# KyleVanMeter/MVOLPS

Hardware: AMD Instinct MI355X
Metric: simplex_pivots_per_s (higher is better)
Workload: dtype f64

## Files before the change

### include/mvx.h

```cpp
#ifndef MVX_H
#define MVX_H

#ifdef __cplusplus
extern "C" {
#endif

#define MVX_MIN 1
#define MVX_MAX 2
#define MVX_CV 1
#define MVX_IV 2
#define MVX_BV 3
#define MVX_FR 1
#define MVX_LO 2
#define MVX_UP 3
#define MVX_DB 4
#define MVX_FX 5
#define MVX_BS 1
#define MVX_NL 2
#define MVX_NU 3
#define MVX_NF 4
#define MVX_NS 5
#define MVX_UNDEF 1
#define MVX_FEAS 2
#define MVX_INFEAS 3
// ... 75 lines not shown
int mvx_gmi_cuts_many(const mvx_prob *const *Ps, int repaired, const int *cols, int count, double *vals, double *rhs, int *ok);
int mvx_classify_many(const mvx_prob *const *Ps, int count, int quirks, int *status, int *nviol, int *viol, double *xviol, int cap);
int mvx_branch_penalties_many(const mvx_prob *const *Ps, int count, const int *cols, const int *col_off, double tol, double *pen_down,
                              double *pen_up, int *arg_down, int *arg_up);
int mvx_round_many(const mvx_prob *root, const mvx_prob *const *Ps, int count, int mode, double *obj, int *found, double *x);
int mvx_rc_tighten_many(const mvx_prob *const *Ps, int count, const double *cutoff, double tol, int *cnt, int *cols, double *lb,
                        double *ub);
int mvx_tighten_cols_many(mvx_prob *const *Ps, int count, const int *off, const int *cols, const double *lb, const double *ub);

int mvx_get_tableau_ld(const mvx_prob *P);
int mvx_get_tableau(const mvx_prob *P, double *out);
int mvx_get_basis(const mvx_prob *P, int *head, int *nb, int *flag);

int mvx_device_count(void);
int mvx_set_device(int dev);
void mvx_profile_enable(int on);
void mvx_profile_reset(void);
double mvx_profile_update_ms(void);
long long mvx_profile_update_launches(void);
double mvx_last_solve_ms(const mvx_prob *P);
long long mvx_pack_size(const mvx_prob *P);
int mvx_pack(const mvx_prob *P, void *dev_buf);
long long mvx_pack_size_from(const mvx_prob *P, const mvx_prob *base);
int mvx_pack_from(const mvx_prob *P, const mvx_prob *base, void *dev_buf);
int mvx_unpack(mvx_prob *dst, const mvx_prob *base, const void *dev_buf);
void mvx_set_tuning(int tr, int hot, int nt);
void mvx_set_refresh(int check_every, double tol);
int mvx_get_refresh_cnt(const mvx_prob *P);
double mvx_row_residual(const mvx_prob *P);
void mvx_set_persist(int mode);
void mvx_set_chain(int len);
void mvx_set_cluster(int on);
void mvx_cluster_stats(long long *launches, long long *aborts);
void mvx_set_dual_chain(int len);
void mvx_persist_stats(long long *launches, long long *aborts);
void mvx_persist_cycles(unsigned long long *out5);
void mvx_set_batch_slots(int slots);
void mvx_sync(void);
int mvx_last_error(void);
int mvx_bind_thread(void);

#ifdef __cplusplus
}
#endif
#endif
```

### mvolps_amd/__init__.py

```python
import ctypes as C
import os

from . import capi

_HERE = os.path.dirname(os.path.abspath(__file__))
LIB_PATH = os.path.join(_HERE, "lib", "libmvolps_amd.so")

_EXTRA = {
    "device_count": (C.c_int, []),
    "set_device": (C.c_int, [C.c_int]),
    "profile_enable": (None, [C.c_int]),
    "profile_reset": (None, []),
    "profile_update_ms": (C.c_double, []),
    "profile_update_launches": (C.c_longlong, []),
    "last_solve_ms": (C.c_double, [C.c_void_p]),
    "sync": (None, []),
    "set_tuning": (None, [C.c_int, C.c_int, C.c_int]),
    "set_batch_slots": (None, [C.c_int]),
    "set_persist": (None, [C.c_int]),
    "set_chain": (None, [C.c_int]),
    "set_cluster": (None, [C.c_int]),
    "cluster_stats": (None, [C.POINTER(C.c_longlong), C.POINTER(C.c_longlong)]),
    "set_dual_chain": (None, [C.c_int]),
    "set_refresh": (None, [C.c_int, C.c_double]),
    "get_refresh_cnt": (C.c_int, [C.c_void_p]),
    "row_residual": (C.c_double, [C.c_void_p]),
    "persist_stats": (None, [C.POINTER(C.c_longlong), C.POINTER(C.c_longlong)]),
    "last_error": (C.c_int, []),
    "bind_thread": (C.c_int, []),
    "persist_cycles": (None, [C.POINTER(C.c_ulonglong)]),
    "simplex_batch": (C.c_int, [C.POINTER(C.c_void_p), C.c_int, C.c_void_p, C.POINTER(C.c_int)]),
    "pack_size": (C.c_longlong, [C.c_void_p]),
    "pack": (C.c_int, [C.c_void_p, C.c_void_p]),
    "pack_size_from": (C.c_longlong, [C.c_void_p, C.c_void_p]),
    "pack_from": (C.c_int, [C.c_void_p, C.c_void_p, C.c_void_p]),
    "unpack": (C.c_int, [C.c_void_p, C.c_void_p, C.c_void_p]),
}

_api = None


def load_library():
    if os.environ.get("MVX_NO_TORCH") != "1":
        try:
            import torch
        except Exception:
            pass
    if not os.path.exists(LIB_PATH):
        raise RuntimeError(
            "libmvolps_amd.so is missing (%s): build it with `python -m mvolps_amd.build`; "
            "there is no fallback path" % LIB_PATH
        )
    return C.CDLL(LIB_PATH)


# ... 19 lines not shown
```

### mvolps_amd/csrc/capi.cpp

```cpp
#include <cfloat>
#include <cmath>
#include <cstdio>
#include <cstdlib>
#include <chrono>
#include <cstring>

#include "engine.hpp"
#include "../../include/mvx_dist.h"

using mvx::RowPtr;

static const double INF = HUGE_VAL;
static int g_term_out = 1;

static void fault(const char *msg) {
  std::fprintf(stderr, "mvx: %s\n", msg);
  std::abort();
}

static void norm_bounds(int type, double lb, double ub, double *olb, double *oub) {
  switch (type) {
    case MVX_FR: *olb = -INF; *oub = INF; break;
    case MVX_LO: *olb = lb; *oub = INF; break;
    case MVX_UP: *olb = -INF; *oub = ub; break;
// ... 471 lines not shown
int mvx_rc_tighten_many(const mvx_prob *const *Ps, int count, const double *cutoff, double tol, int *cnt, int *cols, double *lb,
                        double *ub) {
  return mvx::engine_rc_tighten_many(Ps, count, cutoff, tol, cnt, cols, lb, ub);
}
int mvx_tighten_cols_many(mvx_prob *const *Ps, int count, const int *off, const int *cols, const double *lb, const double *ub) {
  return mvx::engine_tighten_many(Ps, count, off, cols, lb, ub);
}

int mvx_device_count(void) { return mvx::device_count(); }
int mvx_set_device(int dev) { return mvx::set_device(dev); }
long long mvx_pack_size(const mvx_prob *P) { return mvx::engine_pack_size(P, P->m); }
int mvx_pack(const mvx_prob *P, void *dev_buf) { return mvx::engine_pack(P, P->m, dev_buf); }
long long mvx_pack_size_from(const mvx_prob *P, const mvx_prob *base) { return mvx::engine_pack_size(P, base ? base->m : P->m); }
int mvx_pack_from(const mvx_prob *P, const mvx_prob *base, void *dev_buf) { return mvx::engine_pack(P, base ? base->m : P->m, dev_buf); }
int mvx_unpack(mvx_prob *dst, const mvx_prob *base, const void *dev_buf) {
  if (dst == base) return -1;
  mvx::release_device(dst);
  dst->m = base->m; dst->n = base->n; dst->dir = base->dir;
  dst->A = base->A; dst->c = base->c; dst->kind = base->kind; dst->cname = base->cname;
  dst->rtype = base->rtype; dst->rlb = base->rlb; dst->rub = base->rub;
  dst->ctype = base->ctype; dst->clb = base->clb; dst->cub = base->cub;
  dst->valid = false; dst->sol_fresh = false; dst->fresh_rows = -1;
  return mvx::engine_unpack(dst, dev_buf);
}
void mvx_set_tuning(int tr, int hot, int nt) { mvx::tuning(tr, hot, nt); }
void mvx_set_stall_limit(int limit) { mvx::set_stall_limit(limit); }
int mvx_fcs_debug_stamps(unsigned long long *out) { return mvx::fcs_debug_stamps(out); }
void mvx_set_refresh(int check_every, double tol) { mvx::set_refresh(check_every, tol); }
int mvx_get_refresh_cnt(const mvx_prob *P) { return P->refresh_cnt; }
double mvx_row_residual(const mvx_prob *P) { return mvx::row_residual(P); }
void mvx_set_persist(int mode) { mvx::set_persist(mode); }
void mvx_set_chain(int len) { mvx::set_chain(len); }
void mvx_set_cluster(int on) { mvx::set_cluster(on); }
void mvx_cluster_stats(long long *launches, long long *aborts) { mvx::cluster_stats(launches, aborts); }
void mvx_set_dual_chain(int len) { mvx::set_dual_chain(len); }
void mvx_persist_stats(long long *launches, long long *aborts) { mvx::persist_stats(launches, aborts); }
void mvx_persist_cycles(unsigned long long *out5) { mvx::persist_cycles(out5); }
void mvx_set_batch_slots(int slots) { mvx::set_batch_slots(slots); }
void mvx_profile_enable(int on) { mvx::profile_enable(on); }
void mvx_profile_reset(void) { mvx::profile_reset(); }
double mvx_profile_update_ms(void) { return mvx::profile_update_ms(); }
long long mvx_profile_update_launches(void) { return mvx::profile_update_launches(); }
double mvx_last_solve_ms(const mvx_prob *P) { return P->last_ms; }
void mvx_sync(void) { mvx::sync_stream(); }
int mvx_last_error(void) { return mvx::take_last_error(); }
int mvx_bind_thread(void) { return mvx::bind_thread(); }

void *mvx_image_alloc(size_t bytes) { return mvx::engine_image_alloc(bytes); }
void mvx_image_free(void *buf) { mvx::engine_image_free(buf); }
static long long img_pack_size(const void *P, const void *base) { return mvx_pack_size_from((const mvx_prob *)P, (const mvx_prob *)base); }
static int img_pack(const void *P, const void *base, void *buf) { return mvx_pack_from((const mvx_prob *)P, (const mvx_prob *)base, buf); }
static int img_unpack(void *dst, const void *base, const void *buf) { return mvx_unpack((mvx_prob *)dst, (const mvx_prob *)base, buf); }
const mvx_image_api *mvx_hip_image_api(void) {
  static const mvx_image_api t = {img_pack_size, img_pack, img_unpack, mvx_image_alloc, mvx_image_free};
  return &t;
}

}
```

### mvolps_amd/csrc/engine.cpp

```cpp
#include <hip/hip_runtime.h>

#include <cmath>
#include <cstdio>
#include <cstdlib>
#include <cstring>
#include <atomic>
#include <map>
#include <mutex>
#include <tuple>
#include <unordered_map>
#include <vector>

#include "engine.hpp"

struct DevMatrix {
  int m0 = 0, n = 0, lda = 0;
  double *plain = nullptr, *packed = nullptr;
  int *len = nullptr;
  std::vector<const void *> rows;
  ~DevMatrix() {
    if (packed && packed != plain) (void)hipFree(packed);
    if (plain) (void)hipFree(plain);
    if (len) (void)hipFree(len);
  }
};

struct RoundModel {
  int m0 = 0, n = 0, ldm = 0, dir = 0;
  void *dev = nullptr;
  size_t o_rlo = 0, o_rhi = 0, o_clo = 0, o_chi = 0, o_c = 0, o_flags = 0;
  std::vector<mvx::RowPtr> rows;
  std::vector<double> c, clb, cub, rlb, rub;
  std::vector<int> kind;
  ~RoundModel() {
    if (dev) (void)hipFree(dev);
  }
};

namespace mvx {

#define HIPCHECK(expr)                                                                         \
  do {                                                                                         \
    hipError_t e_ = (expr);                                                                    \
    if (e_ != hipSuccess) {                                                                    \
      std::fprintf(stderr, "mvx: HIP error %s at %s:%d (%s)\n", hipGetErrorString(e_), __FILE__, __LINE__, #expr); \
      std::abort();                                                                            \
    }                                                                                          \
  } while (0)

void set_tuning(int tr, int hot, int nt);
int fused_npb(int n);
int fused_nrb_max(int m);
int chain_ncb(int n);
int chain_nrb(int m);
void launch_pboot(const ChainArgs &, hipStream_t);
void launch_pstep(const ChainArgs &, int g, hipStream_t);
void launch_pc(const ChainArgs &, int g, hipStream_t);
void launch_fbc3(const ChainArgs &, int steps, hipStream_t);
void launch_fpatch(const ChainArgs &, int steps, hipStream_t);
int launch_chain(const ChainArgs &, hipStream_t);
int chain_cluster_nw(int m, int n);
int chain_cluster_kmax(int m, int n);
void launch_dboot(Ctl *, int n, hipStream_t);
void launch_da(Ctl *, int n, hipStream_t);
void launch_db(Ctl *, int m, int n, hipStream_t);
void launch_select(Ctl *, hipStream_t, int slots = 1);
int launch_dsel(Ctl *, int m, int n, hipStream_t, int slots = 1);
void launch_select_queue(Ctl *, const BatchQueue &q, hipStream_t, int slots);
void launch_update(Ctl *, int m, int n, hipStream_t, int slots = 1, int chained = 0, int busy_slots = 0);
void launch_p1_head(Ctl *, hipStream_t);
void launch_p1_select(Ctl *, hipStream_t);
void launch_p1_fix(Ctl *, int n, hipStream_t);
void launch_scatter_ctl(Ctl *dst, const Ctl *src, const int *idx, int count, hipStream_t);
void launch_copy_many(const CopyBatch &b, hipStream_t);
void launch_gmi(const GmiArgs &a, hipStream_t);
void launch_classify(const ClsArgs &a, hipStream_t);
void launch_penalty(const PenArgs &a, hipStream_t);
void launch_round(const RndArgs &a, hipStream_t);
void launch_rcfix(const RcArgs &a, hipStream_t);
void launch_tighten(const TightHandle *hs, const TightEntry *es, int count, hipStream_t);
void launch_refresh_select(Ctl *, const int *tflag, int var, hipStream_t);
size_t persist_lds_bytes(int m, int cpw);
int persist_max_cpw();
int persist_slot_words(int m_cap);
int launch_persist(Ctl *, unsigned long long *head, unsigned long long *slot, int *abort_flag, unsigned long long *dbg, int m, int cpw, int nw,
                   int slot_stride, int max_steps, int head_stride, hipStream_t);
void launch_rowcomb(Ctl *, int m, int n, int respect_done, hipStream_t);
void launch_shift_nonbasic(double *T, int ld, int m, int jj, double delta, hipStream_t);
void launch_set_basic_bounds(double *blb, double *bub, int i, double lb, double ub, hipStream_t);
void launch_set_nonbasic(double *nlb, double *nub, int *nflag, int j, double lb, double ub, int flag, hipStream_t);
void launch_add_rows(double *T, int ld, int n, int *bvar, double *blb, double *bub, int *nvar, int first, int nrs, int m_new,
// ... 543 lines not shown
    default: return MVX_NS;
  }
}

static void rebuild_pos(mvx_prob *P) {
  P->pos.assign((size_t)P->m + P->n + 1, 0);
  for (int i = 1; i <= P->m; i++) P->pos[P->bvar[i]] = i;
  for (int j = 1; j <= P->n; j++) P->pos[P->nvar[j]] = -j;
}

static inline void var_bounds(const mvx_prob *P, int k, double *lb, double *ub) {
  if (k <= P->m) {
    *lb = P->rlb[k];
    *ub = P->rub[k];
  } else {
    *lb = P->clb[k - P->m];
    *ub = P->cub[k - P->m];
  }
}

static std::atomic<int> g_cluster{-1};
static std::atomic<bool> g_cluster_broken{false};
static std::atomic<long long> g_cluster_launches{0}, g_cluster_aborts{0};
static bool cluster_wanted() {
  int v = g_cluster.load();
  if (v < 0) {
    const char *e = std::getenv("MVX_CLUSTER");
    v = e ? (std::atoi(e) != 0) : 1;
    g_cluster.store(v);
  }
  return v != 0 && !g_cluster_broken.load();
}

static int g_chain = -1;
static int chain_length(const mvx_prob *P) {
  if (g_chain < 0) {
    const char *e = std::getenv("MVX_CHAIN");
    g_chain = e ? std::max(1, std::min(KCH, std::atoi(e))) : 0;
  }
  if (g_chain > 0) return g_chain;
  const size_t bytes = (size_t)(P->m + 1) * (size_t)P->ld * 8;
  if (cluster_wanted() && chain_cluster_kmax(P->m, P->n) > 0) return bytes < ((size_t)24 << 20) ? 16 : 32;
  if (bytes < ((size_t)24 << 20)) return 8;
  return 16;
}

static int g_dchain = -1;
static int dual_chain_length(bool wide, bool on_chip = false) {
  if (g_dchain < 0) {
    const char *e = std::getenv("MVX_DCHAIN");
    g_dchain = e ? std::max(1, std::min(DCH_MAX, std::atoi(e))) : 0;
  }
  if (g_dchain > 0) return g_dchain;
  if (on_chip) return 8;
  return wide ? 8 : 4;
}

static void fill_ctl(SolveCtx &sc, mvx_prob *P, Ctl *h) {
  std::memset(h, 0, sizeof(Ctl));
  h->T = P->d_T;
  h->bvar = P->d_bvar; h->blb = P->d_blb; h->bub = P->d_bub;
  h->nvar = P->d_nvar; h->nflag = P->d_nflag; h->nlb = P->d_nlb; h->nub = P->d_nub;
  h->colq = sc.d_colq; h->srow = sc.d_srow; h->cost1 = sc.d_cost1; h->wts = sc.d_wts;
  h->gflag = sc.d_gflag; h->part = sc.d_part; h->rc_base = nullptr; h->rc_out = sc.d_cost1;
  h->m = P->m; h->n = P->n; h->ld = P->ld; h->m_cap = P->m_cap;
  h->sgn = (P->dir == MVX_MAX) ? 1.0 : -1.0;
// ... 364 lines not shown
    if (J.profiled) HIPCHECK(hipEventRecord(c.ev_pool[J.ev_used++], sc.stream));
  };
  int depth;
  if (J.try_fused) depth = std::max(0, std::min(batch, remaining));
  else depth = std::max(1, std::min(batch, remaining));
  auto body = [&](int m_grid) {
    if (J.try_fused) {
      PersistPlan pl;
      if (depth > 0 && !J.profiled && J.resident && !(J.cluster && !g_cluster_broken.load()) && persist_plan(c, P, &pl) && ensure_persist(c, sc, P, pl)) {
        launch_select(sc.d_ctl, sc.stream);
        launch_update(sc.d_ctl, m_grid, n, sc.stream, 1, 1);
        HIPCHECK(hipMemcpyAsync(sc.p_backup, P->slab, P->slab_bytes, hipMemcpyDeviceToDevice, sc.stream));
        HIPCHECK(hipMemcpyAsync(sc.d_pctl, sc.d_ctl, sizeof(Ctl), hipMemcpyDeviceToDevice, sc.stream));
        HIPCHECK(hipMemcpyAsync(sc.d_ppw, sc.d_pw[0], (size_t)P->ld * 8, hipMemcpyDeviceToDevice, sc.stream));
        HIPCHECK(hipMemcpyAsync(sc.d_ppw + P->ld, sc.d_pw[1], (size_t)P->ld * 8, hipMemcpyDeviceToDevice, sc.stream));
        const int head_stride = 4;
        HIPCHECK(hipMemsetAsync(sc.d_pcand, 0, (size_t)2 * pl.nw * head_stride * 8, sc.stream));
        const int steps = 1 << 24;
        if (launch_persist(sc.d_ctl, sc.d_pcand, sc.d_pmsg, sc.d_pabort, (unsigned long long *)(sc.d_pabort + 16), P->m, pl.cpw, pl.nw, sc.p_msg_words, steps, head_stride, sc.stream) == 0) {
          J.persist_queued = true;
          g_persist_launches++;
          launch_select(sc.d_ctl, sc.stream);
          launch_update(sc.d_ctl, m_grid, n, sc.stream, 1, 1);
        } else {
          g_persist_broken = true;
        }
      } else {
        const size_t e_generic = J.ev_used;
        if (J.profiled) J.ev_used += 2;
        if (depth > 0) {
          const bool cl = J.cluster && !g_cluster_broken.load();
          if (!cl) launch_pboot(J.cargs, sc.stream);
          bool first = true;
          const int kc = cl ? std::max(1, std::min(J.chain0, chain_cluster_kmax(m, n))) : std::max(1, J.chain);
          auto chain_launch = [&](int steps) {
            J.cargs.kmax = steps;
            J.cargs.boot = first ? 1 : 0;
            first = false;
            J.cargs.tagbase = sc.xtag;
            sc.xtag += 128;
            if (launch_chain(J.cargs, sc.stream) != 0) g_cluster_broken.store(true);
            g_cluster_launches++;
          };
          for (int left = depth; left > 0;) {
            const int steps = std::min(kc, left);
            if (cl) chain_launch(steps);
            else
              for (int t = 0; t < steps; t++) launch_pstep(J.cargs, t, sc.stream);
            ev();
            launch_fbc3(J.cargs, steps, sc.stream);
            ev();
            launch_fpatch(J.cargs, steps, sc.stream);
            left -= steps;
          }
          if (J.parm.it_lim >= 0 && depth >= remaining && !cl) launch_pc(J.cargs, 0, sc.stream);
        }
        launch_select(sc.d_ctl, sc.stream);
        if (J.profiled) HIPCHECK(hipEventRecord(c.ev_pool[e_generic], sc.stream));
        launch_update(sc.d_ctl, m_grid, n, sc.stream, 1, 1);
        if (J.profiled) HIPCHECK(hipEventRecord(c.ev_pool[e_generic + 1], sc.stream));
      }
    } else if (J.try_dfused) {
      launch_select(sc.d_ctl, sc.stream);
      launch_update(sc.d_ctl, m_grid, n, sc.stream, 1, 1);
      if (depth > 1) {
        launch_dboot(sc.d_ctl, n, sc.stream);
        launch_db(sc.d_ctl, m_grid, n, sc.stream);
        for (int k = 0; k < depth - 1; k++) {
          launch_da(sc.d_ctl, n, sc.stream);
          launch_db(sc.d_ctl, m_grid, n, sc.stream);
        }
      }
    } else {
      for (int k = 0; k < depth; k++) {
        launch_dsel(sc.d_ctl, m, n, sc.stream);
        launch_select(sc.d_ctl, sc.stream);
        ev();
        launch_update(sc.d_ctl, m_grid, n, sc.stream, 1, 1);
        ev();
      }
    }
    launch_export(sc.d_ctl, sc.d_stage, m_grid, n, 0, sc.stream);
    stage_copy_async(sc, P);
  };
  body(m);
// ... 1454 lines not shown
  dst->pending.clear();
  dst->valid = false;
  if (h.valid) {
    SlabLayout L = slab_layout((int)h.m_cap, (int)h.ld);
    void *slab = slab_alloc(c, L.total);
    if (!slab) return -2;
    bind_slab(dst, slab, (int)h.m_cap, (int)h.ld);
    const size_t tb = (size_t)(m + 1) * dst->ld * 8;
    HIPCHECK(hipMemcpyAsync(dst->d_T, d + h.host_bytes, tb, hipMemcpyDeviceToDevice, sc.stream));
    HIPCHECK(hipMemcpyAsync((unsigned char *)slab + L.o_bvar, d + h.host_bytes + align_up(tb, 256), L.total - L.o_bvar,
                            hipMemcpyDeviceToDevice, sc.stream));
    HIPCHECK(hipStreamSynchronize(sc.stream));
    rebuild_pos(dst);
    dst->valid = true;
  }
  return 0;
}

void tuning(int tr, int hot, int nt) {
  sync_stream();
  set_tuning(tr, hot, nt);
  if (g_ctx) {
    g_ctx->main.sc_m_cap = 0;
    g_ctx->main.sc_ld = 0;
  }
}

void set_dual_chain(int len) { g_dchain = (len <= 0) ? 0 : std::min(DCH_MAX, len); }
void set_chain(int len) { g_chain = (len <= 0) ? 0 : std::min(KCH, len); }
void set_cluster(int on) {
  g_cluster.store(on != 0);
  g_cluster_broken.store(false);
}
void cluster_stats(long long *launches, long long *aborts) {
  *launches = g_cluster_launches.load();
  *aborts = g_cluster_aborts.load();
}
void set_persist(int mode) {
  g_persist_mode = mode < 0 ? -1 : (mode > 2 ? 2 : mode);
  g_persist_broken = false;
}
void persist_stats(long long *launches, long long *aborts) {
  *launches = g_persist_launches;
  *aborts = g_persist_aborts;
}
void persist_cycles(unsigned long long *out5) {
  for (int k = 0; k < 48; k++) out5[k] = 0;
  if (!g_ctx || !g_ctx->main.h_pabort) return;
  const unsigned long long *d = (const unsigned long long *)(g_ctx->main.h_pabort + 16);
  for (int k = 0; k < 48; k++) out5[k] = d[k];
}
int fcs_debug_stamps(unsigned long long *out) {
  Context &c = ctx();
  if (!c.main.h_ctl || !c.main.h_ctl->dbg) return 0;
  HIPCHECK(hipDeviceSynchronize());
  HIPCHECK(hipMemcpy(out, c.main.h_ctl->dbg, (size_t)KCH * 16 * 8, hipMemcpyDeviceToHost));
  return KCH;
}
void set_stall_limit(int limit) { g_stall_limit = limit > 0 ? limit : 0; }
void set_batch_slots(int k) { g_batch_slots = k < 2 ? 2 : (k > 256 ? 256 : k); }
void profile_enable(int on) { ctx().prof = on != 0; }
void profile_reset() {
  Context &c = ctx();
  MAIN_LOCK(c);
  c.prof_update_ms = 0.0;
  c.prof_update_n = 0;
// ... 6 lines not shown
```

### mvolps_amd/csrc/engine.hpp

```cpp
#pragma once
#include "mvx_internal.hpp"

namespace mvx {

int device_count();
int set_device(int dev);
void sync_stream();
int take_last_error();
int bind_thread();

int engine_simplex(mvx_prob *P, const mvx_smcp *parm);
int engine_simplex_batch(mvx_prob **probs, int count, const mvx_smcp *parm, int *rcs);

void engine_apply_bounds(mvx_prob *P, int k, int type, double old_lb, double old_ub, double lb, double ub);
void engine_add_rows(mvx_prob *P, int first, int nrs);
void engine_row_from_model(mvx_prob *P, int i);
void engine_recompute_cost_row(mvx_prob *P);
void engine_invalidate(mvx_prob *P);

void engine_copy(mvx_prob *dst, const mvx_prob *src);
void release_device(mvx_prob *P);

void refresh_solution(const mvx_prob *P);
int engine_get_tableau(const mvx_prob *P, double *out);
int engine_get_row(const mvx_prob *P, int row, double *out);

int engine_gmi_cuts(const mvx_prob *P, int mode, const int *cols, int count, double *vals, double *rhs, int *ok);
int engine_gmi_cuts_many(const mvx_prob *const *Ps, int mode, const int *cols, int count, double *vals, double *rhs, int *ok);

int engine_classify_many(const mvx_prob *const *Ps, int count, int quirks, int *status, int *nviol, int *viol, double *xviol, int cap);
int engine_penalties_many(const mvx_prob *const *Ps, int count, const int *cols, const int *col_off, double tol, double *pen_down,
                          double *pen_up, int *arg_down, int *arg_up);
int engine_round_many(const mvx_prob *root, const mvx_prob *const *Ps, int count, int mode, double *obj, int *found, double *x);
int engine_rc_tighten_many(const mvx_prob *const *Ps, int count, const double *cutoff, double tol, int *cnt, int *cols, double *lb,
                           double *ub);
int engine_tighten_many(mvx_prob *const *Ps, int count, const int *off, const int *cols, const double *lb, const double *ub);

long long engine_pack_size(const mvx_prob *P, int m_base);
int engine_pack(const mvx_prob *P, int m_base, void *dev_buf);
int engine_unpack(mvx_prob *dst, const void *dev_buf);
void *engine_image_alloc(size_t bytes);
void engine_image_free(void *p);
void tuning(int tr, int hot, int nt);
void set_stall_limit(int limit);
int fcs_debug_stamps(unsigned long long *out);
void set_persist(int mode);
void set_chain(int len);
void set_cluster(int on);
void cluster_stats(long long *launches, long long *aborts);
void set_dual_chain(int len);
void set_refresh(int check_every, double tol);
double row_residual(const mvx_prob *P);
void persist_stats(long long *launches, long long *aborts);
void persist_cycles(unsigned long long *out5);
void set_batch_slots(int k);
void profile_enable(int on);
void profile_reset();
double profile_update_ms();
long long profile_update_launches();

}
```

### mvolps_amd/csrc/kernels.hip

```cpp
#include <hip/hip_runtime.h>

#include <cmath>
#include <cstdlib>

#include "mvx_internal.hpp"

namespace mvx {

#define TIDX ((int)threadIdx.x)

__device__ __forceinline__ double xdiv(double a, double b) {
  const double q = a / b;
  const double aq = fabs(q);
  if (!(aq > 1e-290 && aq < 1e290)) return q;
  const double r = fma(-q, b, a);
  if (r == 0.0) return q;
  const bool up = (r > 0.0) == (b > 0.0);
  long long bits = __double_as_longlong(q);
  bits += ((q > 0.0) == up) ? 1 : -1;
  const double q1 = __longlong_as_double(bits);
  const double r1 = fma(-q1, b, a);
  return (fabs(r1) < fabs(r)) ? q1 : q;
}

// ... 2608 lines not shown
  }
  if (g == 0 && fresh) {
#pragma unroll
    for (int u = 0; u < CPT; u++) {
      if (jj[u] <= n) {
        A.pw[0][jj[u]] = 1.0;
        A.pw[1][jj[u]] = 1.0;
      }
    }
  }
  if (g > 0) {
    const int xf = g & 1;
#pragma unroll
    for (int u = 0; u < CPT; u++) {
      if (jj[u] <= n) {
        A.drowk[xf][jj[u]] = d[u];
        A.pwk[xf][jj[u]] = wgt[u];
      }
    }
    if (lead) {
      A.drowk[xf][0] = z;
      A.pwk[xf][0] = 1.0;
    }
  }
  if (lead) {
    c->pc_n = g;
    if (g > 0) {
      c->phase = PH_PRIMAL2;
      c->pc_itlim = end_itlim ? 1 : 0;
    }
  }
}

__device__ void chain_commit(const ChainArgs &A, Ctl *c, int nch) {
  __shared__ int s_cp[KCH], s_cq[KCH], s_ck[KCH], s_rf[KCH], s_cf[KCH], s_R[KCH], s_C[KCH];
  const int t = TIDX;
  const bool on = (t < nch);
  int kind = 0, p = 0, q = 0;
  if (on) {
    kind = c->ch_kind[t];
    p = c->ch_p[t];
    q = c->ch_q[t];
    s_ck[t] = kind;
    s_cp[t] = p;
    s_cq[t] = q;
    s_R[t] = (kind == ST_PIVOT) ? c->bvar[p] : 0;
    s_C[t] = (kind == ST_PIVOT) ? c->nvar[q] : 0;
  }
  __syncthreads();
  bool lastrow = true, lastcol = true, lastflag = true;
  if (on) {
    int rf = t, cf = t;
    for (int u = t - 1; u >= 0; u--) {
      if (s_ck[u] != ST_PIVOT) continue;
      if (s_cp[u] == p) rf = u;
      if (s_cq[u] == q) cf = u;
    }
    s_rf[t] = rf;
    s_cf[t] = cf;
    for (int u = t + 1; u < nch; u++) {
      if (s_cq[u] == q) lastflag = false;
      if (s_ck[u] != ST_PIVOT) continue;
      if (s_cp[u] == p) lastrow = false;
      if (s_cq[u] == q) lastcol = false;
    }
  }
  __syncthreads();
  if (t == 0) {
    for (int u = 0; u < nch; u++) {
      if (s_ck[u] != ST_PIVOT) continue;
      const int a = s_rf[u], b = s_cf[u];
      const int kv = s_R[a];
      s_R[a] = s_C[b];
      s_C[b] = kv;
    }
  }
  __syncthreads();
  if (on) {
    if (kind == ST_PIVOT) {
      if (lastrow) {
        c->bvar[p] = s_R[s_rf[t]];
        A.blb[p] = c->ch_elb[t];
        A.bub[p] = c->ch_eub[t];
      }
      if (lastcol) {
        c->nvar[q] = s_C[s_cf[t]];
        A.nlb[q] = c->ch_llb[t];
        A.nub[q] = c->ch_lub[t];
      }
    }
    if (lastflag) A.nflag[q] = c->ch_lf[t];
  }
  if (t == 0) {
    const int piv_n = c->ch_cnt[nch - 1];
    c->it_cnt += piv_n;
    c->n_flips += nch - piv_n;
    c->n_bulk++;
    if (c->budget > 0) c->budget -= piv_n;
    c->stall = c->ch_stall[nch - 1];
    c->pc_epoch++;
  }
}

typedef const double __attribute__((address_space(4))) *kconst_f64;
template <int TR, int NT>
__global__ __launch_bounds__(256) void k_fbc3(const ChainArgs A) {
  __shared__ double s_cq[KCH][TR];
  Ctl *const c = A.c;
  if (c->done != D_RUN || c->fstate != F_RUN) return;
  const int nch = c->pc_n;
  if (nch == 0) return;
  const int n = A.n;
  const size_t ld = (size_t)A.ld;
  const int j0 = 2 * ((int)blockIdx.x * 256 + TIDX);
  const int i0 = 1 + (int)blockIdx.y * TR;
  const int xf = nch & 1;
  const bool act = (j0 <= n);
  const int jc = act ? j0 : 0;
  double *base = A.T + (size_t)i0 * ld + jc;
  double2 v[TR];
#pragma unroll
  for (int r = 0; r < TR; r++) v[r] = ld2<NT>(reinterpret_cast<const double2 *>(base + (size_t)r * ld));
  unsigned flips = 0;
  for (int l = 0; l < nch; l++) flips |= (c->ch_kind[l] == ST_FLIP) ? (1u << l) : 0u;
  for (int e = TIDX; e < nch * TR; e += 256) {
    const int l = e / TR, r = e % TR;
    s_cq[l][r] = ((flips >> l) & 1u) ? 0.0 : A.colq0[(size_t)l * A.cstride + i0 + r];
  }
  __syncthreads();
  const double *sp = A.srow0 + jc;
  const double *zp = A.zeros + jc;
  for (int l0 = 0; l0 < nch; l0 += 4) {
    double2 s4[4];
#pragma unroll
    for (int k = 0; k < 4; k++) {
      const int lk = (l0 + k < nch) ? l0 + k : nch - 1;
      s4[k] = *reinterpret_cast<const double2 *>(((flips >> lk) & 1u) ? zp : sp + (size_t)lk * A.sstride);
    }
#pragma unroll
    for (int k = 0; k < 4; k++) {
      if (l0 + k < nch) {
#pragma unroll
        for (int r = 0; r < TR; r++) {
          const double ci = s_cq[l0 + k][r];
          asm("v_fma_f64 %0, -%1, %2, %0" : "+v"(v[r].x) : "v"(ci), "v"(s4[k].x));
          asm("v_fma_f64 %0, -%1, %2, %0" : "+v"(v[r].y) : "v"(ci), "v"(s4[k].y));
        }
      }
    }
  }
  if (act) {
    if (j0 == 0) {
#pragma unroll
      for (int r = 0; r < TR; r++) base[(size_t)r * ld + 1] = v[r].y;
    } else {
#pragma unroll
      for (int r = 0; r < TR; r++) st2<NT>(reinterpret_cast<double2 *>(base + (size_t)r * ld), v[r]);
    }
    if (blockIdx.y == 0) {
      *reinterpret_cast<double2 *>(A.T + j0) = *reinterpret_cast<const double2 *>(A.drowk[xf] + j0);
      const double2 w = *reinterpret_cast<const double2 *>(A.pwk[xf] + j0);
      *reinterpret_cast<double2 *>(A.pw[0] + j0) = w;
      *reinterpret_cast<double2 *>(A.pw[1] + j0) = w;
    }
  }
  if (blockIdx.x == 0 && blockIdx.y == 0) chain_commit(A, c, nch);
}

__global__ __launch_bounds__(256) void k_fpatch(const ChainArgs A, int kmax) {
  __shared__ int s_kind[KCH], s_p[KCH], s_q[KCH];
  __shared__ double s_piv[KCH], s_ip[KCH], s_xq[KCH], s_delta[KCH], s_u[KCH];
  Ctl *const c = A.c;
  if (c->done != D_RUN || c->fstate != F_RUN) return;
  const int nch = c->pc_n;
  if (nch == 0) return;
  const int m = A.m, n = A.n;
  const size_t ld = (size_t)A.ld;
  const int job = (int)blockIdx.y, x = (int)blockIdx.x * 256 + TIDX;
  const int jk = (job < kmax) ? 0 : (job < 2 * kmax) ? 1 : 2;
  const int l = (jk == 0) ? job : (jk == 1) ? job - kmax : -1;
  bool live = (jk == 2) || (l < nch && c->ch_kind[l < nch ? l : 0] == ST_PIVOT);
  const int span = (jk == 0) ? n : (jk == 1) ? m : A.mcap1 - 1;
  if ((int)blockIdx.x * 256 > span) live = false;
  if (live) {
    const int lp = (l >= 0) ? c->ch_p[l] : 0, lq = (l >= 0) ? c->ch_q[l] : 0;
    if (TIDX < KCH) {
      const int t = (TIDX < nch) ? TIDX : nch - 1;
      const int kind = c->ch_kind[t];
      const double piv = c->ch_piv[t];
      s_kind[TIDX] = kind;
      s_p[TIDX] = c->ch_p[t];
      s_q[TIDX] = c->ch_q[t];
      s_piv[TIDX] = piv;
      s_ip[TIDX] = (kind == ST_PIVOT) ? xdiv(1.0, piv) : 0.0;
      s_xq[TIDX] = c->ch_xq[t];
      s_delta[TIDX] = c->ch_delta[t];
      s_u[TIDX] = (jk == 0) ? A.colq0[(size_t)t * A.cstride + lp] : A.srow0[(size_t)t * A.sstride + (jk == 1 ? lq : 0)];
    }
    const int xc = (x >= 1 && x <= span) ? x : 1;
    double op[KCH];
#pragma unroll
    for (int t = 0; t < KCH; t++) {
      const int tc = (t < nch) ? t : nch - 1;
      op[t] = (jk == 0) ? A.srow0[(size_t)tc * A.sstride + xc] : A.colq0[(size_t)tc * A.cstride + xc];
    }
    double *dst = (jk == 0) ? A.T + (size_t)lp * ld + xc : A.T + (size_t)xc * ld + (jk == 1 ? lq : 0);
    double val = (jk == 2) ? *dst : 0.0;
    __syncthreads();
    const int i = (jk == 0) ? lp : xc, j = (jk == 0) ? xc : (jk == 1) ? lq : 0;
    const int l0 = (jk == 2) ? 0 : l;
#pragma unroll
    for (int t = 0; t < KCH; t++) {
      if (t >= l0 && t < nch) {
        const double ci = (jk == 0) ? s_u[t] : op[t], sj = (jk == 0) ? op[t] : s_u[t];
        if (s_kind[t] == ST_FLIP) {
          if (j == 0) val = fma(ci, s_delta[t], val);
        } else if (i == s_p[t]) {
          val = (j == s_q[t]) ? s_ip[t] : (j == 0) ? s_xq[t] - sj : -sj;
        } else if (j == s_q[t]) {
          val = xdiv(ci, s_piv[t]);
        } else {
          val = fma(-ci, sj, val);
        }
      }
    }
    if (x >= 1 && x <= span) {
      if (jk != 2 || x <= m) *dst = val;
      if (jk == 2) A.betab[x] = val;
    }
  }
}

__device__ __forceinline__ bool row_violation(double beta, double lb, double ub, double tol, double &viol, int &up) {
  viol = 0.0;
  up = 0;
  if (lb > -INFINITY && beta < lb - tol * (1.0 + fabs(lb))) viol = lb - beta;
  if (ub < INFINITY && beta > ub + tol * (1.0 + fabs(ub))) {
    viol = beta - ub;
    up = 1;
  }
  return viol > 0.0;
}

__device__ __forceinline__ bool dual_ratio_col(double a, double d, int f, int to_upper, double tp, int j, Cand &x) {
  if (f == MVX_NS) return false;
  const double aa = to_upper ? -a : a;
  double r;
  if (aa > tp && (f == MVX_NL || f == MVX_NF)) r = (f == MVX_NF) ? fabs(d) : (d < 0.0 ? -d : 0.0);
  else if (aa < -tp && (f == MVX_NU || f == MVX_NF)) r = (f == MVX_NF) ? fabs(d) : (d > 0.0 ? d : 0.0);
  else return false;
  const double mag = fabs(a);
  x = Cand{xdiv(r, mag), mag, j, 0};
  return true;
}

__global__ __launch_bounds__(DA_THREADS) void k_dboot(Ctl *c) {
  __shared__ Cand lds[17];
  const bool lead = (blockIdx.x == 0 && TIDX == 0);
  if (c->done != D_RUN || c->phase != PH_DUAL || c->stall >= c->stall_limit || c->perturbed) {
    if (lead) c->fstate = F_OFF;
    return;
  }
  const int a = c->curA & 1, m = c->m, n = c->n;
// ... 1108 lines not shown
int chain_cluster_nw(int m, int n) {
  const int span = m > n ? m : n;
  int nw = (span + 255) / 256;
  if (nw > 32) nw = 32;
  return nw < 1 ? 1 : nw;
}
int chain_cluster_kmax(int m, int n) {
  const int nw = chain_cluster_nw(m, n), tt = nw * 256;
  const int cpt = (n + tt - 1) / tt, rpt = (m + tt - 1) / tt;
  if (cpt > 2 || rpt > 2) return 0;
  const int per_step = (cpt > 1 || rpt > 1 ? 4 : 2) * 256 * 8;
  const int k = (140 * 1024) / per_step;
  return k > KCH ? KCH : k;
}
int launch_chain(const ChainArgs &a, hipStream_t s) {
  const int tt = a.nw * 256;
  const int cpt = (a.n + tt - 1) / tt, rpt = (a.m + tt - 1) / tt;
  const bool wide = (cpt > 1 || rpt > 1);
  const size_t lds = (size_t)(a.kmax > 0 ? a.kmax : 1) * (wide ? 4 : 2) * 256 * 8;
  static size_t attr1 = 0, attr2 = 0;
  size_t &attr = wide ? attr2 : attr1;
  const void *fn = wide ? reinterpret_cast<const void *>(k_chain<2, 2>) : reinterpret_cast<const void *>(k_chain<1, 1>);
  if (lds > attr) {
    if (hipFuncSetAttribute(fn, hipFuncAttributeMaxDynamicSharedMemorySize, (int)lds) != hipSuccess) {
      (void)hipGetLastError();
      return -1;
    }
    attr = lds;
  }
  if (wide) hipLaunchKernelGGL((k_chain<2, 2>), dim3(8 * a.nw), dim3(256), lds, s, a);
  else hipLaunchKernelGGL((k_chain<1, 1>), dim3(8 * a.nw), dim3(256), lds, s, a);
  return 0;
}
void launch_fpatch(const ChainArgs &a, int steps, hipStream_t s) {
  const int span = a.mcap1 > a.n + 1 ? a.mcap1 : a.n + 1;
  hipLaunchKernelGGL(k_fpatch, dim3((span + 255) / 256, 2 * steps + 1), dim3(256), 0, s, a, steps);
}
void launch_fbc3(const ChainArgs &a, int steps, hipStream_t s) {
  const int m = a.m, n = a.n;
  const int pairs = (n + 2) / 2;
  int tr = pick_tr(m, n);
  if (tr > 16) tr = 16;
  if (!g_tr && tr == 16 && steps >= 12) tr = 8;
  const int nt = pick_nt(m, n);
  dim3 grid((pairs + 255) / 256, (m + tr - 1) / tr);
#define FBC2_CASE(TR_, NT_) \
  if (tr == TR_ && nt == NT_) { hipLaunchKernelGGL((k_fbc3<TR_, NT_>), grid, dim3(256), 0, s, a); return; }
  FBC2_CASE(16, 0) FBC2_CASE(16, 1) FBC2_CASE(16, 2) FBC2_CASE(8, 0) FBC2_CASE(8, 1) FBC2_CASE(8, 2) FBC2_CASE(4, 0) FBC2_CASE(4, 1) FBC2_CASE(4, 2)
#undef FBC2_CASE
  std::abort();
}
void launch_dboot(Ctl *d_ctl, int n, hipStream_t s) { hipLaunchKernelGGL(k_dboot, dim3((n + DA_THREADS) / DA_THREADS), dim3(DA_THREADS), 0, s, d_ctl); }
void launch_da(Ctl *d_ctl, int n, hipStream_t s) { hipLaunchKernelGGL(k_da, dim3((n + DA_THREADS) / DA_THREADS), dim3(DA_THREADS), 0, s, d_ctl); }
void launch_db(Ctl *d_ctl, int m, int n, hipStream_t s) {
  const int pairs = (n + 2) / 2;
  const int tr = pick_tr(m, n);
  const int nt = pick_nt(m, n);
  dim3 grid((pairs + 255) / 256, (m + tr - 1) / tr);
#define DB_CASE(TR_, NT_) \
  if (tr == TR_ && nt == NT_) { hipLaunchKernelGGL((k_fb<TR_, 1, NT_, 1>), grid, dim3(256), 0, s, d_ctl); return; }
  DB_CASE(16, 0) DB_CASE(16, 1) DB_CASE(8, 0) DB_CASE(8, 1) DB_CASE(4, 0) DB_CASE(4, 1) DB_CASE(32, 0) DB_CASE(32, 1)
  DB_CASE(16, 2) DB_CASE(8, 2) DB_CASE(4, 2) DB_CASE(32, 2)
#undef DB_CASE
  std::abort();
}
int launch_dsel(Ctl *d_ctl, int m, int n, hipStream_t s, int slots) {
  static int state = -1;
  if (state < 0) {
    const char *e = std::getenv("MVX_DSEL");
    if (e && e[0] == '0') state = 0;
    else if (hipFuncSetAttribute(reinterpret_cast<const void *>(k_dsel), hipFuncAttributeMaxDynamicSharedMemorySize, (int)DSEL_LDS) == hipSuccess) state = 1;
    else {
      (void)hipGetLastError();
      state = 0;
    }
  }
  if (state != 1 || m > 1024 || n > 1024) return 0;
  hipLaunchKernelGGL(k_dsel, dim3(1, 1, slots), dim3(1024), DSEL_LDS, s, d_ctl);
  return 1;
}
// ... 91 lines not shown
```

Baseline: 58580.

## Fuse chain patch jobs into the batched tableau update kernel

Folds the separate patch kernel's work (pivot rows, pivot columns and beta fixups) into extra leading blocks of the fbc3 rank-update launch. This removes one kernel launch per chain. The update blocks now work out which rows and columns are pivot targets and skip storing them, so the patch blocks can write those entries without racing. It also adds atomic pass-statistics collection in chain_commit and an env/API toggle, with the fused path on by default. The risks are correctness if the patch and update writes overlap, plus some extra per-block ballot work and global atomics.

```diff
diff --git a/include/mvx.h b/include/mvx.h
--- a/include/mvx.h
+++ b/include/mvx.h
@@ -131,6 +131,8 @@
 void mvx_set_chain(int len);
 void mvx_set_cluster(int on);
 void mvx_cluster_stats(long long *launches, long long *aborts);
+void mvx_set_fused_patch(int on);
+void mvx_pass_stats(unsigned *cases, unsigned *lens, int reset);
 void mvx_set_dual_chain(int len);
 void mvx_persist_stats(long long *launches, long long *aborts);
 void mvx_persist_cycles(unsigned long long *out5);
diff --git a/mvolps_amd/__init__.py b/mvolps_amd/__init__.py
--- a/mvolps_amd/__init__.py
+++ b/mvolps_amd/__init__.py
@@ -21,6 +21,8 @@
     "set_chain": (None, [C.c_int]),
     "set_cluster": (None, [C.c_int]),
     "cluster_stats": (None, [C.POINTER(C.c_longlong), C.POINTER(C.c_longlong)]),
+    "set_fused_patch": (None, [C.c_int]),
+    "pass_stats": (None, [C.POINTER(C.c_uint), C.POINTER(C.c_uint), C.c_int]),
     "set_dual_chain": (None, [C.c_int]),
     "set_refresh": (None, [C.c_int, C.c_double]),
     "get_refresh_cnt": (C.c_int, [C.c_void_p]),
diff --git a/mvolps_amd/csrc/capi.cpp b/mvolps_amd/csrc/capi.cpp
--- a/mvolps_amd/csrc/capi.cpp
+++ b/mvolps_amd/csrc/capi.cpp
@@ -527,6 +527,8 @@
 void mvx_set_persist(int mode) { mvx::set_persist(mode); }
 void mvx_set_chain(int len) { mvx::set_chain(len); }
 void mvx_set_cluster(int on) { mvx::set_cluster(on); }
+void mvx_set_fused_patch(int on) { mvx::set_fused_patch(on); }
+void mvx_pass_stats(unsigned *cases, unsigned *lens, int reset) { mvx::pass_stats(cases, lens, reset); }
 void mvx_cluster_stats(long long *launches, long long *aborts) { mvx::cluster_stats(launches, aborts); }
 void mvx_set_dual_chain(int len) { mvx::set_dual_chain(len); }
 void mvx_persist_stats(long long *launches, long long *aborts) { mvx::persist_stats(launches, aborts); }
diff --git a/mvolps_amd/csrc/engine.cpp b/mvolps_amd/csrc/engine.cpp
--- a/mvolps_amd/csrc/engine.cpp
+++ b/mvolps_amd/csrc/engine.cpp
@@ -56,7 +56,8 @@
 void launch_pboot(const ChainArgs &, hipStream_t);
 void launch_pstep(const ChainArgs &, int g, hipStream_t);
 void launch_pc(const ChainArgs &, int g, hipStream_t);
-void launch_fbc3(const ChainArgs &, int steps, hipStream_t);
+void launch_fbc3(const ChainArgs &, int steps, hipStream_t, bool with_patch);
+void pass_stats(unsigned *cases, unsigned *lens, int reset);
 void launch_fpatch(const ChainArgs &, int steps, hipStream_t);
 int launch_chain(const ChainArgs &, hipStream_t);
 int chain_cluster_nw(int m, int n);
@@ -666,6 +667,17 @@
   return v != 0 && !g_cluster_broken.load();
 }
 
+static std::atomic<int> g_fused_patch{-1};
+static bool fused_patch_wanted() {
+  int v = g_fused_patch.load();
+  if (v < 0) {
+    const char *e = std::getenv("MVX_FUSED_PATCH");
+    v = e ? (std::atoi(e) != 0) : 1;
+    g_fused_patch.store(v);
+  }
+  return v != 0;
+}
+
 static int g_chain = -1;
 static int chain_length(const mvx_prob *P) {
   if (g_chain < 0) {
@@ -1096,6 +1108,7 @@
           const bool cl = J.cluster && !g_cluster_broken.load();
           if (!cl) launch_pboot(J.cargs, sc.stream);
           bool first = true;
+          const bool fused_patch = fused_patch_wanted();
           const int kc = cl ? std::max(1, std::min(J.chain0, chain_cluster_kmax(m, n))) : std::max(1, J.chain);
           auto chain_launch = [&](int steps) {
             J.cargs.kmax = steps;
@@ -1112,9 +1125,9 @@
             else
               for (int t = 0; t < steps; t++) launch_pstep(J.cargs, t, sc.stream);
             ev();
-            launch_fbc3(J.cargs, steps, sc.stream);
+            launch_fbc3(J.cargs, steps, sc.stream, fused_patch);
             ev();
-            launch_fpatch(J.cargs, steps, sc.stream);
+            if (!fused_patch) launch_fpatch(J.cargs, steps, sc.stream);
             left -= steps;
           }
           if (J.parm.it_lim >= 0 && depth >= remaining && !cl) launch_pc(J.cargs, 0, sc.stream);
@@ -2635,6 +2648,7 @@
   g_cluster.store(on != 0);
   g_cluster_broken.store(false);
 }
+void set_fused_patch(int on) { g_fused_patch.store(on != 0); }
 void cluster_stats(long long *launches, long long *aborts) {
   *launches = g_cluster_launches.load();
   *aborts = g_cluster_aborts.load();
diff --git a/mvolps_amd/csrc/engine.hpp b/mvolps_amd/csrc/engine.hpp
--- a/mvolps_amd/csrc/engine.hpp
+++ b/mvolps_amd/csrc/engine.hpp
@@ -47,6 +47,8 @@
 void set_persist(int mode);
 void set_chain(int len);
 void set_cluster(int on);
+void set_fused_patch(int on);
+void pass_stats(unsigned *cases, unsigned *lens, int reset);
 void cluster_stats(long long *launches, long long *aborts);
 void set_dual_chain(int len);
 void set_refresh(int check_every, double tol);
diff --git a/mvolps_amd/csrc/kernels.hip b/mvolps_amd/csrc/kernels.hip
--- a/mvolps_amd/csrc/kernels.hip
+++ b/mvolps_amd/csrc/kernels.hip
@@ -2664,6 +2664,8 @@
   }
 }
 
+enum : unsigned { PC_COL1 = 1, PC_COLPAIR = 2, PC_ROWS_CLOSE = 4, PC_ROW_TWICE = 8, PC_FLIP_INSIDE = 16 };
+__device__ unsigned g_pass_stats[2];
 __device__ void chain_commit(const ChainArgs &A, Ctl *c, int nch) {
   __shared__ int s_cp[KCH], s_cq[KCH], s_ck[KCH], s_rf[KCH], s_cf[KCH], s_R[KCH], s_C[KCH];
   const int t = TIDX;
@@ -2683,11 +2685,18 @@
   bool lastrow = true, lastcol = true, lastflag = true;
   if (on) {
     int rf = t, cf = t;
+    unsigned seen = (kind == ST_PIVOT && q == 1) ? PC_COL1 : (kind == ST_FLIP && nch > 1) ? PC_FLIP_INSIDE : 0u;
     for (int u = t - 1; u >= 0; u--) {
       if (s_ck[u] != ST_PIVOT) continue;
       if (s_cp[u] == p) rf = u;
       if (s_cq[u] == q) cf = u;
-    }
+      if (kind != ST_PIVOT) continue;
+      if (s_cq[u] != q && (s_cq[u] >> 1) == (q >> 1)) seen |= PC_COLPAIR;
+      if (s_cp[u] != p && ((s_cp[u] - 1) >> 2) == ((p - 1) >> 2)) seen |= PC_ROWS_CLOSE;
+      if (s_cp[u] == p) seen |= PC_ROW_TWICE;
+    }
+    if (seen) atomicOr(&g_pass_stats[0], seen);
+    if (t == 0) atomicOr(&g_pass_stats[1], 1u << (nch - 1));
     s_rf[t] = rf;
     s_cf[t] = cf;
     for (int u = t + 1; u < nch; u++) {
@@ -2734,86 +2743,15 @@
   }
 }
 
-typedef const double __attribute__((address_space(4))) *kconst_f64;
-template <int TR, int NT>
-__global__ __launch_bounds__(256) void k_fbc3(const ChainArgs A) {
-  __shared__ double s_cq[KCH][TR];
-  Ctl *const c = A.c;
-  if (c->done != D_RUN || c->fstate != F_RUN) return;
-  const int nch = c->pc_n;
-  if (nch == 0) return;
-  const int n = A.n;
-  const size_t ld = (size_t)A.ld;
-  const int j0 = 2 * ((int)blockIdx.x * 256 + TIDX);
-  const int i0 = 1 + (int)blockIdx.y * TR;
-  const int xf = nch & 1;
-  const bool act = (j0 <= n);
-  const int jc = act ? j0 : 0;
-  double *base = A.T + (size_t)i0 * ld + jc;
-  double2 v[TR];
-#pragma unroll
-  for (int r = 0; r < TR; r++) v[r] = ld2<NT>(reinterpret_cast<const double2 *>(base + (size_t)r * ld));
-  unsigned flips = 0;
-  for (int l = 0; l < nch; l++) flips |= (c->ch_kind[l] == ST_FLIP) ? (1u << l) : 0u;
-  for (int e = TIDX; e < nch * TR; e += 256) {
-    const int l = e / TR, r = e % TR;
-    s_cq[l][r] = ((flips >> l) & 1u) ? 0.0 : A.colq0[(size_t)l * A.cstride + i0 + r];
-  }
-  __syncthreads();
-  const double *sp = A.srow0 + jc;
-  const double *zp = A.zeros + jc;
-  for (int l0 = 0; l0 < nch; l0 += 4) {
-    double2 s4[4];
-#pragma unroll
-    for (int k = 0; k < 4; k++) {
-      const int lk = (l0 + k < nch) ? l0 + k : nch - 1;
-      s4[k] = *reinterpret_cast<const double2 *>(((flips >> lk) & 1u) ? zp : sp + (size_t)lk * A.sstride);
-    }
-#pragma unroll
-    for (int k = 0; k < 4; k++) {
-      if (l0 + k < nch) {
-#pragma unroll
-        for (int r = 0; r < TR; r++) {
-          const double ci = s_cq[l0 + k][r];
-          asm("v_fma_f64 %0, -%1, %2, %0" : "+v"(v[r].x) : "v"(ci), "v"(s4[k].x));
-          asm("v_fma_f64 %0, -%1, %2, %0" : "+v"(v[r].y) : "v"(ci), "v"(s4[k].y));
-        }
-      }
-    }
-  }
-  if (act) {
-    if (j0 == 0) {
-#pragma unroll
-      for (int r = 0; r < TR; r++) base[(size_t)r * ld + 1] = v[r].y;
-    } else {
-#pragma unroll
-      for (int r = 0; r < TR; r++) st2<NT>(reinterpret_cast<double2 *>(base + (size_t)r * ld), v[r]);
-    }
-    if (blockIdx.y == 0) {
-      *reinterpret_cast<double2 *>(A.T + j0) = *reinterpret_cast<const double2 *>(A.drowk[xf] + j0);
-      const double2 w = *reinterpret_cast<const double2 *>(A.pwk[xf] + j0);
-      *reinterpret_cast<double2 *>(A.pw[0] + j0) = w;
-      *reinterpret_cast<double2 *>(A.pw[1] + j0) = w;
-    }
-  }
-  if (blockIdx.x == 0 && blockIdx.y == 0) chain_commit(A, c, nch);
-}
-
-__global__ __launch_bounds__(256) void k_fpatch(const ChainArgs A, int kmax) {
+__device__ __forceinline__ void fpatch_job(const ChainArgs &A, Ctl *c, int nch, int jk, int l, int bx) {
   __shared__ int s_kind[KCH], s_p[KCH], s_q[KCH];
   __shared__ double s_piv[KCH], s_ip[KCH], s_xq[KCH], s_delta[KCH], s_u[KCH];
-  Ctl *const c = A.c;
-  if (c->done != D_RUN || c->fstate != F_RUN) return;
-  const int nch = c->pc_n;
-  if (nch == 0) return;
   const int m = A.m, n = A.n;
   const size_t ld = (size_t)A.ld;
-  const int job = (int)blockIdx.y, x = (int)blockIdx.x * 256 + TIDX;
-  const int jk = (job < kmax) ? 0 : (job < 2 * kmax) ? 1 : 2;
-  const int l = (jk == 0) ? job : (jk == 1) ? job - kmax : -1;
+  const int x = bx * 256 + TIDX;
   bool live = (jk == 2) || (l < nch && c->ch_kind[l < nch ? l : 0] == ST_PIVOT);
   const int span = (jk == 0) ? n : (jk == 1) ? m : A.mcap1 - 1;
-  if ((int)blockIdx.x * 256 > span) live = false;
+  if (bx * 256 > span) live = false;
   if (live) {
     const int lp = (l >= 0) ? c->ch_p[l] : 0, lq = (l >= 0) ? c->ch_q[l] : 0;
     if (TIDX < KCH) {
@@ -2861,6 +2799,120 @@
       if (jk == 2) A.betab[x] = val;
     }
   }
+}
+
+__host__ __device__ inline int fbc3_nbr(int n) { return n / 256 + 1; }
+__host__ __device__ inline int fbc3_nbc(int m) { return m / 256 + 1; }
+__host__ __device__ inline int fbc3_nb0(int mcap1) { return (mcap1 - 1) / 256 + 1; }
+template <int TR, int NT>
+__global__ __launch_bounds__(256) void k_fbc3(const ChainArgs A, int npatch, int kj, int ntx) {
+  __shared__ double s_cq[KCH][TR];
+  Ctl *const c = A.c;
+  if (c->done != D_RUN || c->fstate != F_RUN) return;
+  const int nch = c->pc_n;
+  if (nch == 0) return;
+  int b = (int)blockIdx.x;
+  if (b < npatch) {
+    const int nbr = fbc3_nbr(A.n), nbc = fbc3_nbc(A.m);
+    int jk = 0, nb = nbr;
+    if (b >= kj * nbr) {
+      b -= kj * nbr;
+      jk = (b < kj * nbc) ? 1 : 2;
+      nb = nbc;
+    }
+    if (jk == 2) fpatch_job(A, c, nch, 2, -1, b - kj * nbc);
+    else fpatch_job(A, c, nch, jk, b / nb, b % nb);
+    return;
+  }
+  b -= npatch;
+  const int tx = b % ntx, ty = b / ntx;
+  const int n = A.n;
+  const size_t ld = (size_t)A.ld;
+  const int j0 = 2 * (tx * 256 + TIDX);
+  const int i0 = 1 + ty * TR;
+  const int xf = nch & 1;
+  const bool act = (j0 <= n);
+  const int jc = act ? j0 : 0;
+  double *base = A.T + (size_t)i0 * ld + jc;
+  double2 v[TR];
+#pragma unroll
+  for (int r = 0; r < TR; r++) v[r] = ld2<NT>(reinterpret_cast<const double2 *>(base + (size_t)r * ld));
+  const int lt = TIDX & 31, lc = (lt < nch) ? lt : nch - 1;
+  const int kind_l = c->ch_kind[lc], p_l = c->ch_p[lc], q_l = c->ch_q[lc];
+  const bool piv_l = (lt < nch) && (kind_l == ST_PIVOT);
+  const unsigned flips = (unsigned)__ballot((lt < nch) && (kind_l == ST_FLIP));
+  unsigned rmask = 0;
+#pragma unroll
+  for (int r = 0; r < TR; r++) rmask |= __ballot(piv_l && p_l == i0 + r) ? (1u << r) : 0u;
+  const int jw = j0 - 2 * (TIDX & 63);
+  unsigned chit = (unsigned)__ballot(piv_l && (unsigned)(q_l - jw) < 128u);
+  unsigned cm = (j0 == 0) ? 1u : 0u;
+  while (chit) {
+    const int l = __ffs(chit) - 1;
+    chit &= chit - 1;
+    const int q = __builtin_amdgcn_readlane(q_l, l);
+    if ((q >> 1) == (j0 >> 1)) cm |= 1u << (q & 1);
+  }
+  const bool plain = (__ballot(cm != 0) == 0);
+  for (int e = TIDX; e < nch * TR; e += 256) {
+    const int l = e / TR, r = e % TR;
+    s_cq[l][r] = ((flips >> l) & 1u) ? 0.0 : A.colq0[(size_t)l * A.cstride + i0 + r];
+  }
+  __syncthreads();
+  const double *sp = A.srow0 + jc;
+  const double *zp = A.zeros + jc;
+  for (int l0 = 0; l0 < nch; l0 += 4) {
+    double2 s4[4];
+#pragma unroll
+    for (int k = 0; k < 4; k++) {
+      const int lk = (l0 + k < nch) ? l0 + k : nch - 1;
+      s4[k] = *reinterpret_cast<const double2 *>(((flips >> lk) & 1u) ? zp : sp + (size_t)lk * A.sstride);
+    }
+#pragma unroll
+    for (int k = 0; k < 4; k++) {
+      if (l0 + k < nch) {
+#pragma unroll
+        for (int r = 0; r < TR; r++) {
+          const double ci = s_cq[l0 + k][r];
+          asm("v_fma_f64 %0, -%1, %2, %0" : "+v"(v[r].x) : "v"(ci), "v"(s4[k].x));
+          asm("v_fma_f64 %0, -%1, %2, %0" : "+v"(v[r].y) : "v"(ci), "v"(s4[k].y));
+        }
+      }
+    }
+  }
+  if (act) {
+    if (plain) {
+#pragma unroll
+      for (int r = 0; r < TR; r++)
+        if (!((rmask >> r) & 1u)) st2<NT>(reinterpret_cast<double2 *>(base + (size_t)r * ld), v[r]);
+    } else {
+#pragma unroll
+      for (int r = 0; r < TR; r++) {
+        if ((rmask >> r) & 1u) continue;
+        if (cm == 0) st2<NT>(reinterpret_cast<double2 *>(base + (size_t)r * ld), v[r]);
+        else if (cm == 1) base[(size_t)r * ld + 1] = v[r].y;
+        else if (cm == 2) base[(size_t)r * ld] = v[r].x;
+      }
+    }
+    if (ty == 0) {
+      *reinterpret_cast<double2 *>(A.T + j0) = *reinterpret_cast<const double2 *>(A.drowk[xf] + j0);
+      const double2 w = *reinterpret_cast<const double2 *>(A.pwk[xf] + j0);
+      *reinterpret_cast<double2 *>(A.pw[0] + j0) = w;
+      *reinterpret_cast<double2 *>(A.pw[1] + j0) = w;
+    }
+  }
+  if (b == 0) chain_commit(A, c, nch);
+}
+
+__global__ __launch_bounds__(256) void k_fpatch(const ChainArgs A, int kmax) {
+  Ctl *const c = A.c;
+  if (c->done != D_RUN || c->fstate != F_RUN) return;
+  const int nch = c->pc_n;
+  if (nch == 0) return;
+  const int job = (int)blockIdx.y;
+  const int jk = (job < kmax) ? 0 : (job < 2 * kmax) ? 1 : 2;
+  const int l = (jk == 0) ? job : (jk == 1) ? job - kmax : -1;
+  fpatch_job(A, c, nch, jk, l, (int)blockIdx.x);
 }
 
 __device__ __forceinline__ bool row_violation(double beta, double lb, double ub, double tol, double &viol, int &up) {
@@ -4035,20 +4087,35 @@
   else hipLaunchKernelGGL((k_chain<1, 1>), dim3(8 * a.nw), dim3(256), lds, s, a);
   return 0;
 }
+void pass_stats(unsigned *cases, unsigned *lens, int reset) {
+  unsigned h[2] = {0, 0};
+  (void)hipMemcpyFromSymbol(h, HIP_SYMBOL(g_pass_stats), sizeof h);
+  *cases = h[0];
+  *lens = h[1];
+  if (reset) {
+    h[0] = h[1] = 0;
+    (void)hipMemcpyToSymbol(HIP_SYMBOL(g_pass_stats), h, sizeof h);
+  }
+}
 void launch_fpatch(const ChainArgs &a, int steps, hipStream_t s) {
   const int span = a.mcap1 > a.n + 1 ? a.mcap1 : a.n + 1;
   hipLaunchKernelGGL(k_fpatch, dim3((span + 255) / 256, 2 * steps + 1), dim3(256), 0, s, a, steps);
 }
-void launch_fbc3(const ChainArgs &a, int steps, hipStream_t s) {
+static int fbc3_patch_blocks(const ChainArgs &a, int steps) {
+  return steps * (fbc3_nbr(a.n) + fbc3_nbc(a.m)) + fbc3_nb0(a.mcap1);
+}
+void launch_fbc3(const ChainArgs &a, int steps, hipStream_t s, bool with_patch) {
   const int m = a.m, n = a.n;
   const int pairs = (n + 2) / 2;
   int tr = pick_tr(m, n);
   if (tr > 16) tr = 16;
   if (!g_tr && tr == 16 && steps >= 12) tr = 8;
   const int nt = pick_nt(m, n);
-  dim3 grid((pairs + 255) / 256, (m + tr - 1) / tr);
+  const int ntx = (pairs + 255) / 256, nty = (m + tr - 1) / tr;
+  const int npatch = with_patch ? fbc3_patch_blocks(a, steps) : 0;
+  dim3 grid((unsigned)(npatch + ntx * nty));
 #define FBC2_CASE(TR_, NT_) \
-  if (tr == TR_ && nt == NT_) { hipLaunchKernelGGL((k_fbc3<TR_, NT_>), grid, dim3(256), 0, s, a); return; }
+  if (tr == TR_ && nt == NT_) { hipLaunchKernelGGL((k_fbc3<TR_, NT_>), grid, dim3(256), 0, s, a, npatch, steps, ntx); return; }
   FBC2_CASE(16, 0) FBC2_CASE(16, 1) FBC2_CASE(16, 2) FBC2_CASE(8, 0) FBC2_CASE(8, 1) FBC2_CASE(8, 2) FBC2_CASE(4, 0) FBC2_CASE(4, 1) FBC2_CASE(4, 2)
 #undef FBC2_CASE
   std::abort();
```

Measured after the change: 47180. 0.805x the previous value.
